# YukeWang96/GNNAdvisor_OSDI21

Hardware: AMD Instinct MI355X
Metric: aggregated edges/sec, GCN sum-aggregation SpMM (SAG) hidden=64 (higher is better)
Workload: dtype f32; 1 GPU; reddit-like power-law graph, random node order; num_nodes=232965, nnz=114623790, dim=64, partSize=128, num_parts=1008217, parallelism=single GPU, call=GNNA.SAG (pybind module, reference signature, fresh output), decider=auto/mi355x, column_phases=16, build_id=0.6.1+df1c895dd0a4406b

## Files before the change

### gnnadvisor_osdi21_amd/_lib.py

```python
from __future__ import annotations

import ctypes
import math
import os

import torch

_HERE = os.path.dirname(os.path.abspath(__file__))
LIB_PATH = os.environ.get("GNNA_LIB") or os.path.join(_HERE, "csrc", "libgnna.so")

GNNA_OK = 0


class GnnaError(RuntimeError):
    pass


class Tuning(ctypes.Structure):
    _fields_ = [("struct_size", ctypes.c_int), ("groups_per_chunk", ctypes.c_int), ("loads_in_flight", ctypes.c_int),
                ("blocks_per_cu", ctypes.c_int), ("xcd_remap", ctypes.c_int),
                ("trust_canonical", ctypes.c_int), ("column_phases", ctypes.c_int),
                ("avg_degree", ctypes.c_int), ("nonlocal_ids", ctypes.c_int), ("gcn_prescale", ctypes.c_int),
                ("pad_rows", ctypes.c_int), ("zero_fill", ctypes.c_int),
                ("sweep", ctypes.c_int), ("sweep_slack", ctypes.c_int), ("deterministic", ctypes.c_int),
# ... 47 lines not shown
    "gnna_release_graph": (i, [p]), "gnna_forget_graph": (i, [p]), "gnna_forget_plans": (i, [p]),
    "gnna_runtime_counters": (None, [pi64]),
    "gnna_runtime_counters_ex": (i, [pi64, i]),
    "gnna_debug_untrusted_copies": (i, [p]),
    "gnna_profile_begin": (i, [i]),
    "gnna_profile_end": (i, [pd, pd, pi]),
    "gnna_agg_edge_ld_f32": (i, [p, i64, i64, p, p, p, p, p] + _SIZES),
    "gnna_edge_softmax_f32": (i, [p, p, i64, i64, i, p, p]),
    "gnna_edge_softmax_backward_f32": (i, [p, p, p, i64, i64, i, p, p]),
    "gnna_reverse_edges_i32": (i, [p, p, i64, p]),
    "gnna_agg_reduce_ld_f32": (i, [i, p, i64, i64, p, p, p, p, i64, p] + _SIZES),
    "gnna_scatter_arg_ld_f32": (i, [p, i64, p, i64, p, i64, p, i64, i64, i, u, p]),
    "gnna_gat_forward_f32": (i, _GAT_FWD + [i64, i, i, i64, i, u, p]),
    "gnna_gat_forward_rect_f32": (i, _GAT_FWD + [i64, i64, i, i, i64, i, u, p]),
    "gnna_gat_backward_f32": (i, _GAT_BWD + [p, p, p, p, f, p, i64, p, p, i64, i, i, i64, i, u, p]),
    "gnna_gat_backward_dir_f32": (i, _GAT_BWD + _GAT_BOTH + [i64, i, i, i, u, p]),
    "gnna_gat_backward_rect_f32": (i, _GAT_BWD + _GAT_BOTH + [i64, i64, i, i, i, u, p]),
    "gnna_transpose_csr_i32": (i, [p, p, i64, i64, p, p, p, p]),
    "gnna_count_parts_device_i32": (i64, [i, p, i64, p]),
    "gnna_build_part_device_i32": (i, [i, p, i64, p, p, i64, p]),
    "gnna_sample_neighbors_i32": (i, [p, p, i64, p, i64, i, u64, i, p, p, p, p, p, p, i64, i64, pi64, p]),
    "gnna_agg_typed_expand_ld_f32": (i, _TYPED),
    "gnna_agg_typed_contract_ld_f32": (i, _TYPED),
    "gnna_typed_coef_grad_ld_f32": (i, [p, i64, i64, p, i64, i64, p, p, p, p, p, p, i, i, i, i64, i, u, p]),
}
EXT_SIGNATURES = {
    "gnna_gat_forward_drop_f32": (i, _GAT_FWD[:9] + [f, u64] + _GAT_FWD[9:] + [i64, i64, i, i, i64, i, u, p]),
    "gnna_gat_backward_drop_f32": (i, _GAT_BWD + _GAT_BOTH[:11] + [f, u64] + _GAT_BOTH[11:] + [i64, i64, i, i, i, u, p]),
}
_GRAPH_T = ([p] * 4 + [i64]) * 2
GATV2_SIGNATURES = {
    "gnna_gatv2_forward_f32": (i, [p, i64, p, i64, p] + [p] * 4 + [f, f, u64, p, i64, p, i64, i64, i, i, i64, i, u, p]),
    "gnna_gatv2_backward_f32": (i, [p, i64, p, i64, p, p, p, i64, p, i64] + _GRAPH_T + [f, f, u64, p, i64, p, i64, p,
                                                                                       i64, i64, i, i, i, u, p]),
}
DOTATTN_SIGNATURES = {
    "gnna_dot_attn_forward_f32": (i, [p, i64] * 3 + [p] * 4 + [f, f, u64, p, i64, p, i64, i64, i, i, i64, i, u, p]),
    "gnna_dot_attn_backward_f32": (i, [p, i64] * 3 + [p, p, i64, p, i64] + _GRAPH_T + [f, f, u64] + [p, i64] * 3 +
                                   [i64, i64, i, i, i, u, p]),
}
GATEDGE_SIGNATURES = {
    "gnna_gat_edge_forward_f32": (i, _GAT_FWD[:4] + [p] + _GAT_FWD[4:9] + [f, u64] + _GAT_FWD[9:] + [i64, i64, i64, i, i, i64, i, u, p]),
    "gnna_gat_edge_backward_f32": (i, _GAT_BWD[:4] + [p] + _GAT_BWD[4:] + _GAT_BOTH[:10] + [p, f, f, u64] + _GAT_BOTH[11:] +
                                   [p, i64, i64, i64, i, i, i, u, p]),
    "gnna_gat_alpha_f32": (i, [p] * 6 + [f, p, i64, i64, i64, i, p]),
}
STATS_SIGNATURES = {
    "gnna_agg_stats_ld_f32": (i, [p, i64, i64, p, p, p] + [p, i64] * 6 + [i64, i, i64, i, u, p]),
}
SOFTAGG_SIGNATURES = {
    "gnna_agg_softmax_ld_f32": (i, [p, i64, i64, p, i, p, p] + [p, i64] * 3 + [i64, i, u, p]),
    "gnna_agg_softmax_backward_ld_f32": (i, [p, i64, i64, p, i] + [p, i64] * 3 + [p, p, p, i64, i64, i, u, p]),
}
del p, i, i64, u, u64, f, s, pd, pi, pi64
EXPORTS = tuple(SIGNATURES)
EXT_EXPORTS = tuple(EXT_SIGNATURES)
GATV2_EXPORTS = tuple(GATV2_SIGNATURES)
DOTATTN_EXPORTS = tuple(DOTATTN_SIGNATURES)
SIGNATURE_TABLES = (SIGNATURES, EXT_SIGNATURES, GATV2_SIGNATURES, DOTATTN_SIGNATURES)
GATEDGE_EXPORTS = tuple(GATEDGE_SIGNATURES)
STATS_EXPORTS = tuple(STATS_SIGNATURES)
LATER_SIGNATURE_TABLES = (GATEDGE_SIGNATURES, STATS_SIGNATURES)
SOFTAGG_EXPORTS = tuple(SOFTAGG_SIGNATURES)
NEWER_SIGNATURE_TABLES = (SOFTAGG_SIGNATURES,)


def load() -> ctypes.CDLL:
    global _lib
    if _lib is not None:
        return _lib
    if not os.path.exists(LIB_PATH):
        raise ImportError(
            f"{LIB_PATH} is missing: the HIP extension has not been built "
            "(run `python -m gnnadvisor_osdi21_amd.build`). There is no CPU fallback.")
    L = ctypes.CDLL(LIB_PATH)
    for table in SIGNATURE_TABLES + LATER_SIGNATURE_TABLES + NEWER_SIGNATURE_TABLES:
        for name, (restype, argtypes) in table.items():
            fn = getattr(L, name)
            fn.restype = restype
            if argtypes is not None:
                fn.argtypes = argtypes
    _lib = L
    return L


def _check(rc: int) -> None:
    if rc != GNNA_OK:
        raise GnnaError(f"libgnna error {rc}: {load().gnna_last_error().decode()}")


def _ptr(t: torch.Tensor | None) -> int | None:
    return None if t is None else t.data_ptr()


def _stream(device: torch.device) -> int:
    return torch.cuda.current_stream(device).cuda_stream


def _call(device, fn_name: str, *args) -> None:
    with torch.cuda.device(device):
        _check(getattr(load(), fn_name)(*args, _stream(device)))


def _need_device(t: torch.Tensor, what: str) -> None:
    if not t.is_cuda:
        raise GnnaError(f"{what} needs device tensors: there is no CPU path in libgnna")


def set_tuning(groups_per_chunk=-1, loads_in_flight=-1, blocks_per_cu=-1, xcd_remap=-1,
               trust_canonical=-1, column_phases=-1, avg_degree=-1, nonlocal_ids=-1, gcn_prescale=-1,
               pad_rows=-1, zero_fill=-1, sweep=-1, sweep_slack=-1, deterministic=-1, pack_ids=-1,
               wide_blocks=-1, ids_check_every=-1) -> None:
    t = Tuning(ctypes.sizeof(Tuning), groups_per_chunk, loads_in_flight, blocks_per_cu, xcd_remap, trust_canonical, column_phases,
               avg_degree, nonlocal_ids, gcn_prescale, pad_rows, zero_fill, sweep, sweep_slack, deterministic,
               pack_ids, ids_check_every, wide_blocks)
    _check(load().gnna_set_tuning(ctypes.byref(t)))


def reset_tuning() -> None:
    _check(load().gnna_set_tuning(None))


def device_cus() -> int:
    return int(load().gnna_device_cus())


def host_threads() -> int:
    return int(load().gnna_host_threads())

# ... 88 lines not shown


def degrees(row_pointers: torch.Tensor) -> torch.Tensor:
    rp = _host_i32(row_pointers)
    out = torch.empty(rp.numel() - 1, dtype=torch.float32)
    _check(load().gnna_degrees_f32(rp.data_ptr(), rp.numel() - 1, out.data_ptr()))
    return out


def edge_span(src, dst) -> float:
    s, d = _host_i32(src), _host_i32(dst)
    v = ctypes.c_double()
    _check(load().gnna_edge_span(s.data_ptr(), d.data_ptr(), s.numel(), ctypes.byref(v)))
    return v.value


def _reorder(entry: str, src, dst, num_nodes: int) -> torch.Tensor:
    s, d = _host_i32(src), _host_i32(dst)
    out = torch.empty(int(num_nodes), dtype=torch.int32)
    _check(getattr(load(), entry)(s.data_ptr(), d.data_ptr(), s.numel(), int(num_nodes), out.data_ptr()))
    return out


def reorder_rcm(src, dst, num_nodes: int) -> torch.Tensor:
    return _reorder("gnna_reorder_rcm_i32", src, dst, num_nodes)


def reorder_community(src, dst, num_nodes: int) -> torch.Tensor:
    return _reorder("gnna_reorder_community_i32", src, dst, num_nodes)


def reorder_community_csr(row_pointers, column_index, num_nodes: int) -> torch.Tensor:
    rp, ci = _host_i32(row_pointers), _host_i32(column_index)
    assert rp.numel() == int(num_nodes) + 1
    out = torch.empty(int(num_nodes), dtype=torch.int32)
    _check(load().gnna_reorder_community_csr_i32(rp.data_ptr(), ci.data_ptr(), int(num_nodes), out.data_ptr()))
    return out


def relabel_edges_(src: torch.Tensor, dst: torch.Tensor, new_id: torch.Tensor, num_nodes: int) -> float:
    for t in (src, dst, new_id):
        assert t.dtype == torch.int32 and t.is_contiguous() and not t.is_cuda
    v = ctypes.c_double()
    _check(load().gnna_relabel_edges_i32(src.data_ptr(), dst.data_ptr(), src.numel(), new_id.data_ptr(), int(num_nodes), ctypes.byref(v)))
    return v.value


def relabel_csr(row_pointers, column_index, new_id, num_nodes: int):
    rp, ci, nid = _host_i32(row_pointers), _host_i32(column_index), _host_i32(new_id)
    out_rp = torch.empty(int(num_nodes) + 1, dtype=torch.int32)
    out_ci = torch.empty(max(1, ci.numel()), dtype=torch.int32)
    _check(load().gnna_relabel_csr_i32(rp.data_ptr(), ci.data_ptr(), int(num_nodes), nid.data_ptr(), out_rp.data_ptr(), out_ci.data_ptr()))
    return out_rp, out_ci[:ci.numel()]


def last_num_phases() -> int:
    return int(load().gnna_last_num_phases())


def last_num_launches() -> int:
    return int(load().gnna_last_num_launches())


def profile_begin(max_calls: int) -> None:
    _check(load().gnna_profile_begin(int(max_calls)))


def profile_end() -> dict:
    a, b, n = ctypes.c_double(), ctypes.c_double(), ctypes.c_int()
    _check(load().gnna_profile_end(ctypes.byref(a), ctypes.byref(b), ctypes.byref(n)))
    return dict(main_ms=a.value, prologue_ms=b.value, calls=n.value)


def count_parts(partSize: int, indptr: torch.Tensor) -> int:
    assert indptr.dtype == torch.int32 and not indptr.is_cuda and indptr.is_contiguous()
    n = load().gnna_count_parts(int(partSize), indptr.data_ptr(), indptr.numel() - 1)
    if n < 0:
        _check(int(n))
    return int(n)


def build_part(partSize: int, indptr: torch.Tensor):
    indptr = indptr.contiguous()
    P = count_parts(partSize, indptr)
    pp = torch.empty(P + 1, dtype=torch.int32)
    p2n = torch.empty(P, dtype=torch.int32)
    _check(load().gnna_build_part_i32(int(partSize), indptr.data_ptr(), indptr.numel() - 1,
                                      pp.data_ptr(), p2n.data_ptr(), P))
    return pp, p2n


def _fresh_output(shape, device, dtype=torch.float32) -> torch.Tensor:
    if os.environ.get("GNNA_DEBUG_POISON", "0") not in ("", "0"):
        return torch.full(tuple(shape), float("nan") if dtype.is_floating_point else -(2 ** 31), dtype=dtype, device=device)
    return torch.empty(tuple(shape), dtype=dtype, device=device)


def _agg(fn_name, X, row_pointers, column_index, extra, part_pointers, part2Node, partSize, dimWorker,
         warpPerBlock, out):
    _need_device(X, "aggregation")
    assert X.dtype == torch.float32 and X.is_contiguous() and X.dim() == 2
    for t in (column_index, part_pointers, part2Node):
        assert t.dtype == torch.int32 and t.is_contiguous() and t.device == X.device
    if out is None:
        out = _fresh_output(X.shape, X.device)
    _call(X.device, fn_name, X.data_ptr(), _ptr(row_pointers), column_index.data_ptr(), extra,
# ... 821 lines not shown
```

### gnnadvisor_osdi21_amd/build.py

```python
from __future__ import annotations

import os
import subprocess
import sys
import sysconfig

PKG = os.path.dirname(os.path.abspath(__file__))
ROOT = os.path.dirname(PKG)
CSRC = os.path.join(PKG, "csrc")
INCLUDE = os.path.join(ROOT, "include")
LIB = os.path.join(CSRC, "libgnna.so")
EXT = os.path.join(PKG, "GNNAdvisor.so")
ARCH = "gfx950"
HIPCC = os.environ.get("HIPCC", "/opt/rocm/bin/hipcc")

LIB_SOURCES = [os.path.join(CSRC, f) for f in ("gnna_agg.hip", "gnna_stream.hip", "gnna_sweep.hip", "gnna_x16.hip", "gnna_reduce.hip", "gnna_stats.hip", "gnna_softagg.hip", "gnna_sddmm.hip", "gnna_edge.hip", "gnna_gat.hip", "gnna_gatv2.hip", "gnna_dotattn.hip", "gnna_typed.hip", "gnna_transpose.hip", "gnna_sample.hip",
                                                "gnna_gemm.hip", "gnna_runtime.hip", "gnna_host.cpp", "gnna_reorder.cpp")]
LIB_DEPS = LIB_SOURCES + [os.path.join(CSRC, "gnna_internal.h"), os.path.join(CSRC, "gnna_device.h"), os.path.join(CSRC, "gnna_launch.h"),
                           os.path.join(CSRC, "gnna_gat_common.h"), os.path.join(CSRC, "gnna_keys.h"), os.path.join(INCLUDE, "gnna.h"), os.path.join(INCLUDE, "gnna_ext.h"),
                           os.path.join(INCLUDE, "gnna_gatv2.h"), os.path.join(INCLUDE, "gnna_dotattn.h"),
                           os.path.join(INCLUDE, "gnna_gat_edge.h"), os.path.join(INCLUDE, "gnna_stats.h"),
                           os.path.join(INCLUDE, "gnna_softagg.h")]
EXT_SOURCES = [os.path.join(CSRC, "gnna_torch.cpp")]
EXT_DEPS = EXT_SOURCES + [os.path.join(INCLUDE, "gnna.h"), os.path.join(INCLUDE, "gnna_ext.h"), os.path.join(INCLUDE, "gnna_gatv2.h"),
                          os.path.join(INCLUDE, "gnna_dotattn.h"), os.path.join(INCLUDE, "gnna_gat_edge.h"),
                          os.path.join(INCLUDE, "gnna_stats.h"), os.path.join(INCLUDE, "gnna_softagg.h")]


def source_hash() -> str:
    import hashlib
    h = hashlib.sha256()
    for path in sorted(set(LIB_DEPS + EXT_DEPS)):
        h.update(os.path.relpath(path, ROOT).encode() + b"\0")
        with open(path, "rb") as f:
            h.update(f.read())
        h.update(b"\0")
    return h.hexdigest()[:16]


def _stale(target: str, deps: list[str]) -> bool:
    if not os.path.exists(target):
        return True
    t = os.path.getmtime(target)
    return any(os.path.getmtime(d) > t for d in deps)


def build_lib(force: bool = False, verbose: bool = False) -> str:
    from concurrent.futures import ThreadPoolExecutor
    objdir = os.path.join(CSRC, "build")
    os.makedirs(objdir, exist_ok=True)
    headers = [d for d in LIB_DEPS if d not in LIB_SOURCES]
    flags = [f"--offload-arch={ARCH}", "-O3", "-std=c++17", "-fPIC", "-munsafe-fp-atomics", "-ffp-contract=off",
             "-fvisibility=hidden", "-I" + INCLUDE, "-I" + CSRC]
    jobs, objs = [], []
    digest = source_hash()
    stamp = os.path.join(objdir, "source_hash.txt")
    stamped = open(stamp).read().strip() if os.path.exists(stamp) else ""
    if not force and stamped == digest and os.path.exists(LIB) and not _stale(LIB, LIB_DEPS):
        return LIB
    for src in LIB_SOURCES:
        obj = os.path.join(objdir, os.path.basename(src) + ".o")
        objs.append(obj)
        carries_id = os.path.basename(src) == "gnna_host.cpp"
        if force or _stale(obj, [src] + headers) or (carries_id and stamped != digest):
            jobs.append([HIPCC, *flags, *([f'-DGNNA_SOURCE_HASH="{digest}"'] if carries_id else []), "-c", src, "-o", obj])

    def run(cmd):
        if verbose:
            print(" ".join(cmd), flush=True)
        subprocess.check_call(cmd)
    if jobs:
        with ThreadPoolExecutor(max_workers=min(len(jobs), os.cpu_count() or 4)) as pool:
            list(pool.map(run, jobs))
    if jobs or force or _stale(LIB, objs):
        run([HIPCC, f"--offload-arch={ARCH}", "-shared", "-fPIC", "-fvisibility=hidden", *objs, "-o", LIB])
# ... 45 lines not shown
```

### gnnadvisor_osdi21_amd/csrc/gnna_agg.hip

```cpp
#include <hip/hip_runtime.h>

#include <algorithm>
#include <cmath>
#include <cstdint>
#include <cstdio>

#include "gnna.h"
#include "gnna_device.h"
#include "gnna_internal.h"

namespace gnna {
namespace {


__global__ void __launch_bounds__(kBlock)
prologue_kernel(float *__restrict__ Y, size_t n_floats, int D, int ldy, const int32_t *__restrict__ p2n,
                const int32_t *__restrict__ pp, int64_t P, int32_t *flag, int32_t seq, int validate, int zero_fill,
                const int32_t *__restrict__ chk_ids, int64_t chk_n, const unsigned long long *__restrict__ chk_sum,
                int32_t *stale_flag, uint32_t *__restrict__ clear_words, int n_clear)
{
    if (blockIdx.x == 0 && (int)threadIdx.x < n_clear) clear_words[threadIdx.x] = 0u;
    const unsigned fill_blocks = chk_ids ? gridDim.x - 1 : gridDim.x;
    if (blockIdx.x >= fill_blocks) {
        if (threadIdx.x < kWave) {
// ... 560 lines not shown
                                              "stream capture: run the sequence once before capturing it");
        if (plan.stats.unsorted > 0)
            return fail(GNNA_ERR_UNSUPPORTED, "windowed aggregation: the column ids of %.0f neighbor-groups are not in increasing "
                                              "order (sort the ids of every row, as the loader's CSR has them)", plan.stats.unsorted);
        cnt = plan.cnt; S = plan.S; B = 1;
        win_lo = win_begin; win_hi = win_end == num_windows ? S : win_end;
    } else {
        if (tune.column_phases >= 2 && num_in_rows >= kMaxSlices) {
            B = std::min(tune.column_phases, kMaxSlices);
            rc = get_slice_plan(ds, stream, column_index, part_pointers, part2Node, num_parts, num_in_rows, false, false, &plan);
            if (rc != GNNA_OK) return rc;
        } else if (tune.column_phases == 0 && can_slice && foot_bytes >= ((size_t)6 << 20)) {
            rc = get_slice_plan(ds, stream, column_index, part_pointers, part2Node, num_parts, num_in_rows, true, false, &plan);
            if (rc != GNNA_OK) return rc;
            if (plan.cnt && plan.stats.valid)
                B = choose_slices(plan.stats, foot_bytes, plan.S, plan.slice_rows, num_nodes, num_in_rows == num_nodes,
                                  tune.nonlocal_ids == 1);
        }
        cnt = plan.cnt;
        if (cnt) S = plan.S;
        if (!cnt || B < 2) { B = 1; cnt = nullptr; }
    }

    const int auto_Bs = (cnt && !windowed && plan.stats.valid)
                            ? sweep_auto_phases(tune, mode, dim, foot_bytes, num_nodes, num_in_rows, plan.stats, B, ds->num_cus,
                                                tune.deterministic == 1, partSize) : 0;
    if (mode != MODE_EDGE && cnt && !windowed && dim >= 4 && (tune.sweep == 1 || auto_Bs > 0) && tune.deterministic != 1 &&
        sweep_supports(mode, dim, x_bytes)) {
        int Bs = B;
        if (auto_Bs > 0) {
            Bs = std::min(auto_Bs, S);
        } else if (tune.column_phases < 2) {
            Bs = std::max(2, std::min(std::min(std::min(16, 2 * B), std::max(2, partSize / 4)), S));
        }
        const int32_t *sw_ids = nullptr; const uint32_t *sw_off = nullptr;
        if (plan.handle && (tune.pack_ids == 1 || (tune.pack_ids == 0 && plan.pinned)) && tune.xcd_remap != 0) {
            rc = get_packed_ids(ds, stream, plan.handle, Bs, kWave, true, false, &sw_ids, &sw_off, &chk_sum, &chk_n, stale_flag, seq,
                                tune.ids_check_every);
            if (rc != GNNA_OK) return rc;
            if (sw_ids) count_event(CTR_PACKED_LAUNCHES);
        }
        uint32_t *sync = ds->sweep_sync + (size_t)call_block_of(ds, stream, seq) * kSweepSlotWords;
        static_assert(kXcds * 16 + 2 <= kBlock, "the prologue clears the sweep counters with one block");
        rc = run_prologue(0, sync, kXcds * 16 + 2);
        if (rc != GNNA_OK) return rc;
        SweepLaunch w;
        w.mode = mode; w.X = X; w.col = column_index; w.pp = part_pointers; w.p2n = part2Node; w.Y = out;
        w.cnt = cnt; w.row_scale = row_scale; w.flag = flag; w.seq = seq; w.trust = tune.trust_canonical ? 1 : 0; w.sync = sync;
        w.P = num_parts; w.D = dim; w.ldx = ldx; w.ldy = ldy; w.S = S; w.B = Bs;
        w.relu = relu; w.num_out_rows = num_nodes;
        w.U = std::max(tune.loads_in_flight, 8);
        w.rows_with_edges = plan.stats.valid ? (int64_t)std::min((double)num_nodes, plan.stats.groups) : num_nodes;
        if (tune.groups_per_chunk > 64) w.rounds = tune.groups_per_chunk / 64;
        w.slack = tune.sweep_slack; w.wgs_per_cu = tune.blocks_per_cu;
        w.dynamic = tune.xcd_remap != 0;
        w.plain_ok = !accumulate_into_out; w.eps = eps;
        w.ids_packed = sw_ids; w.item_off = sw_off; w.packed_stale = stale_flag;
        t_last_phases = Bs;
        t_last_launches = 1;
        rc = launch_sweep(ds, w, stream);
        if (rc != GNNA_OK) return rc;
        profile_record(prof_call, 2, stream);
        return GNNA_OK;
    }

    int G = std::min(64, tune.groups_per_chunk * B);
    if (mode == MODE_EDGE && cnt && !windowed && plan.handle && plan.pinned && (plan.stats.valid || tune.sweep == 1) &&
        tune.xcd_remap != 0) {
        const int Bs = sweep_phases_of_width(tune, dim, foot_bytes, x_bytes, num_nodes, num_in_rows, plan.stats, B, ds->num_cus,
                                             partSize, S);
        if (Bs >= 2) { B = Bs; G = kWave; }
    }
    t_last_phases = B;
    StreamLaunch a;
    a.mode = mode; a.X = X; a.col = column_index; a.pp = part_pointers; a.p2n = part2Node; a.Y = out;
    a.cnt = cnt; a.row_scale = row_scale; a.flag = flag; a.seq = seq;
    if (mode == MODE_EDGE) { a.deg_row = nullptr; a.deg_col = nullptr; a.edge_w = degrees_in; }
    else { a.deg_row = degrees; a.deg_col = degrees_in; }
    a.trust = tune.trust_canonical ? 1 : 0; a.P = num_parts;
    a.D = dim; a.ldx = ldx; a.ldy = ldy; a.G = G; a.U = tune.loads_in_flight; a.S = S; a.B = B;
    a.win_lo = win_lo; a.win_hi = win_hi; a.relu = relu; a.num_out_rows = num_nodes;
    t_last_launches = 1;
    a.wide = wide; a.plain_ok = (B == 1 && !accumulate_into_out && !windowed); a.xcd_remap = tune.xcd_remap != 0;
    a.eps = eps;
    if (tune.deterministic == 1 && !windowed) {
        const int G_eff = std::max(1, std::min(a.G, kWave));
        const size_t chunks = (size_t)((num_parts + G_eff - 1) / G_eff);
        const size_t part_bytes = ((chunks * 2 * (size_t)dim * sizeof(float)) + 255) & ~(size_t)255;
        const size_t stamp_bytes = chunks * 2 * sizeof(int32_t);
        void *ws = nullptr;
        rc = get_workspace(ds, stream, 2, part_bytes + stamp_bytes, &ws);
        if (rc != GNNA_OK) return rc;
        a.det = true;
        a.det_part = static_cast<float *>(ws);
        a.det_stamp = reinterpret_cast<int32_t *>(static_cast<char *>(ws) + part_bytes);
        hipError_t em = hipMemsetAsync(a.det_stamp, 0, stamp_bytes, stream);
        if (em != hipSuccess) return fail(GNNA_ERR_HIP, "deterministic schedule scratch: %s", hipGetErrorString(em));
        t_last_launches = B;
    }
    if (cnt && !windowed && plan.handle && (tune.pack_ids == 1 || (tune.pack_ids == 0 && plan.pinned))) {
        rc = get_packed_ids(ds, stream, plan.handle, B, std::max(1, std::min(a.G, kWave)), true, false, &a.ids_packed, &a.item_off,
                            &chk_sum, &chk_n, stale_flag, seq, tune.ids_check_every);
        a.packed_stale = stale_flag;
        if (rc != GNNA_OK) return rc;
        if (a.ids_packed) count_event(CTR_PACKED_LAUNCHES);
    }
    const bool sparse = !a.det && a.plain_ok && tune.zero_fill != 2 &&
// ... 292 lines not shown
```

### gnnadvisor_osdi21_amd/csrc/gnna_internal.h

```cpp
#ifndef GNNA_INTERNAL_H_
#define GNNA_INTERNAL_H_

#include <hip/hip_runtime.h>

#include <atomic>
#include <cstddef>
#include <cstdint>
#include <map>
#include <utility>
#include <vector>

#include "gnna.h"
#include "gnna_launch.h"

namespace gnna {

int fail(int code, const char *fmt, ...) __attribute__((format(printf, 2, 3)));

int host_thread_budget(int cap);

void apply_graph_hints(const void *column_index, int dim, gnna_tuning *tune);

int launch_ok(const char *prefix_fmt, ...) __attribute__((format(printf, 1, 2)));
inline int xcd_remap_on()
// ... 98 lines not shown
       CTR_COUNT = 10 };
void count_event(int which);

struct StreamLaunch {
    int mode;
    const float *X; const int32_t *col; const int32_t *pp; const int32_t *p2n; float *Y;
    const uint8_t *cnt;
    const float *row_scale;
    const float *deg_row; const float *deg_col;
    const float *A = nullptr;
    const float *edge_w = nullptr;
    const int32_t *flag; int32_t seq; int32_t trust;
    int64_t P;
    int D, ldx, G, U, S, B;
    int lda = 0;
    int ldy = 0;
    int win_lo = 0, win_hi = 0;
    bool relu = false;
    int64_t num_out_rows = 0;
    bool wide, plain_ok, xcd_remap;
    float eps;
    bool det = false;
    float *det_part = nullptr; int32_t *det_stamp = nullptr;
    const int32_t *ids_packed = nullptr; const uint32_t *item_off = nullptr;
    const int32_t *packed_stale = nullptr;
};
int launch_stream(const StreamLaunch &a, hipStream_t stream);
int launch_stream_epilogue_only(const StreamLaunch &a, hipStream_t stream);

struct SweepLaunch {
    int mode;
    const float *X; const int32_t *col; const int32_t *pp; const int32_t *p2n; float *Y;
    const uint8_t *cnt;
    const float *row_scale;
    const int32_t *flag; int32_t seq; int32_t trust;
    uint32_t *sync;
    int64_t P;
    int D, ldx, U, S, B;
    int ldy = 0;
    bool relu = false;
    int64_t num_out_rows = 0;
    int rounds = 0;
    int64_t rows_with_edges = 0;
    int slack = 0;
    int wgs_per_cu = 0;
    bool dynamic = true;
    bool plain_ok;
    float eps;
    const int32_t *ids_packed = nullptr; const uint32_t *item_off = nullptr;
    const int32_t *packed_stale = nullptr;
};
bool sweep_supports(int mode, int dim, size_t x_bytes);
int sweep_acc_rows(int dim, int wgs_per_cu);
int launch_sweep(DeviceState *ds, const SweepLaunch &a, hipStream_t stream);
int sweep_auto_phases(const gnna_tuning &t, int mode, int dim, size_t x_bytes, int64_t num_out_rows, int64_t num_in_rows,
                      const SlicePlanStats &st, int B, int num_cus, bool deterministic, int part_size);
constexpr int kSweepListCap = 1023;
constexpr int kSweepSlotWords = 8 * 16 + 2 + 2 * kSweepListCap;

struct X16Launch {
    int mode;
    int in_type, out_type;
    const void *input; int64_t ld_in, num_in_rows;
    const int32_t *column_index; const float *degrees_out; const float *degrees_in; float epsilon;
    const int32_t *part_pointers; const int32_t *part2Node;
    void *out; int64_t ld_out, num_out_rows;
    int dim; int64_t num_parts; int partSize;
    bool accumulate, relu, xcd_remap;
    int prof_call = -1;
};
int launch_x16(DeviceState *ds, hipStream_t stream, const X16Launch &c);
int reserve_x16(DeviceState *ds, hipStream_t stream, int64_t num_in_rows, int64_t num_out_rows, int dim);
int launch_zero_fill(DeviceState *ds, hipStream_t stream, float *out, int64_t rows, int dim, int64_t ld);
void launch_relu_rows(DeviceState *ds, hipStream_t stream, float *out, int64_t rows, int dim, int64_t ld);

int64_t scan_tiles(int64_t n);
int launch_exclusive_scan(hipStream_t stream, int32_t *data, int64_t n, int32_t *partial);
int refuse_capture(const char *what, hipStream_t stream);

int profile_acquire_call(bool has_work);
void profile_record(int call, int which, hipStream_t stream);

}

#endif
```

### gnnadvisor_osdi21_amd/csrc/gnna_sweep.hip

```cpp
#include <hip/hip_runtime.h>

#include <algorithm>
#include <cmath>
#include <cstdint>

#include "gnna.h"
#include "gnna_device.h"
#include "gnna_internal.h"

namespace gnna {
namespace {

constexpr int kSweepIdSlots = 512;
constexpr int kSweepBlock = 1024;
constexpr int kSweepWaves = kSweepBlock / kWave;
constexpr int kSweepLockWords = 128;

template <int LPR, int WGS> constexpr int acc_floats()
{
    return WGS == 1 ? (LPR >= 16 ? 32768 : 28672) : (LPR >= 16 ? 15360 : 11264);
}

__device__ __forceinline__ void lds_add(float *p, float v)
{
    typedef __attribute__((address_space(3))) float lds_float;
    (void)__hip_atomic_fetch_add((lds_float *)p, v, __ATOMIC_RELAXED, __HIP_MEMORY_SCOPE_WORKGROUP);
}

struct SweepParams {
    const float *X;
    const int32_t *col;
    const int32_t *pp;
    const int32_t *p2n;
    float *Y;
    const uint8_t *cnt;
    const float *row_scale;
    const int32_t *flag;
    uint32_t *sync;
    int64_t P;
    int32_t seq;
    int32_t trust;
    int32_t D;
    int32_t ldx;
    int32_t ldy;
    int32_t relu;
    int32_t S;
    int32_t B;
    int32_t rounds;
    int32_t plain_ok;
    int32_t dynamic;
    int32_t slack;
    float eps;
    const int32_t *ids_packed;
    const uint32_t *item_off;
    const int32_t *packed_stale;
    int64_t num_chunks;
};

__device__ __forceinline__ int64_t lower_bound64(const int32_t *__restrict__ pp, int64_t P, int64_t target, int lane)
{
    int64_t lo = 0, hi = P;
    while (hi > lo) {
        const int64_t span = hi - lo;
        const int64_t idx = lo + (span * lane) / kWave;
        const bool below = (int64_t)pp[idx] < target;
        const int c = __popcll(__ballot(below));
        if (c == 0) { hi = lo; break; }
        const int64_t new_lo = lo + (span * (c - 1)) / kWave + 1;
        const int64_t new_hi = c < kWave ? lo + (span * c) / kWave : hi;
        lo = new_lo;
        hi = new_hi > new_lo ? new_hi : new_lo;
    }
    return lo;
}

__device__ __forceinline__ int64_t sweep_set_start(int64_t i, int64_t num_sets, int64_t nnz, const int32_t *__restrict__ pp,
                                                   int64_t P, bool canonical, bool align64, int lane)
{
    const int64_t target = i >= num_sets ? nnz : (nnz * i) / num_sets;
    int64_t g = i <= 0 ? 0 : (i >= num_sets ? P : (canonical ? lower_bound64(pp, P, target, lane) : (P * i) / num_sets));
    if (align64 && g < P) g &= ~(int64_t)(kWave - 1);
    return g;
}

__global__ void __launch_bounds__(kBlock)
sweep_relu_fixup_kernel(float *__restrict__ Y, int64_t N, int D, int ldy, const uint32_t *__restrict__ list,
                        const int32_t *flag, int32_t seq, int32_t trust, int whole)
{
    const int lane = threadIdx.x & (kWave - 1);
    const int64_t wave = ((int64_t)blockIdx.x * blockDim.x + threadIdx.x) >> 6;
    const int64_t nwaves = ((int64_t)gridDim.x * blockDim.x) >> 6;
    const bool canonical = trust || (*flag != seq);
    auto clamp_row = [&](int64_t r) {
        float *row = Y + (size_t)r * (size_t)ldy;
        for (int i = lane; i < D; i += kWave) row[i] = fmaxf(row[i], 0.f);
    };
    if (whole || !canonical || list[1] != 0u) {
        for (int64_t r = wave; r < N; r += nwaves) clamp_row(r);
        return;
    }
    const uint32_t n = list[0] < (uint32_t)kSweepListCap ? list[0] : (uint32_t)kSweepListCap;
    for (int64_t i = wave; i < (int64_t)n; i += nwaves) {
        const int64_t first = (int64_t)list[2 + 2 * i], cnt = (int64_t)list[3 + 2 * i];
        for (int64_t r = first; r < first + cnt && r < N; r++) clamp_row(r);
    }
}

template <int LPR, int MODE, int U, int WGS>
__global__ void __launch_bounds__(kSweepBlock) __attribute__((amdgpu_waves_per_eu(4 * WGS, 4 * WGS)))
sweep_kernel(const SweepParams p)
{
    typedef typename VecOf<4>::T VT;
    typedef typename VecOf<4>::M MT;
    constexpr int RPI = kWave / LPR;
    constexpr int RL = (kSweepIdSlots / RPI < kWave) ? kSweepIdSlots / RPI : kWave;
    static_assert(RL % U == 0, "a round is a whole number of batches");
    constexpr int ACC = acc_floats<LPR, WGS>();
    __shared__ float s_acc[ACC];
    __shared__ uint32_t s_off[kSweepWaves][RL * RPI];
    __shared__ int64_t s_g[2];
    __shared__ int s_ctl[8];
    __shared__ unsigned s_lock[kSweepLockWords];

    const int lane = threadIdx.x & (kWave - 1);
    const int wib = __builtin_amdgcn_readfirstlane((int)threadIdx.x >> 6);
    const int lslot = lane / LPR;
    const int c = lane % LPR;
    const int D = p.D;
    const bool canonical = p.trust || (*p.flag != p.seq);
    const bool stale_ids = p.ids_packed != nullptr && *p.packed_stale == p.seq;
    const char *xbase = reinterpret_cast<const char *>(p.X);
    const uint32_t row_bytes32 = (uint32_t)p.ldx * 4u;
    uint32_t *offs = s_off[wib];
    const int CAP = ACC / D;
    const unsigned long long upto = (2ull << lane) - 1ull;
    const unsigned long long above = ~upto;

    const int piece = c * 4;
    const bool cvalid = piece < D;
    int dcol = piece, shift = 0;
    if (piece + 4 > D && cvalid) { dcol = D - 4; shift = piece - dcol; }
    const uint32_t col_off = (uint32_t)(cvalid ? dcol : 0) * 4u;
    const int comp = lane >> 4;
    const bool add_lane = LPR <= 16 ? ((lane & 15) < LPR && cvalid && comp >= shift) : (lslot == 0 && cvalid);

    const int xcd = (int)(blockIdx.x & (kXcds - 1));
    const int nbx = (int)(gridDim.x >> 3);
    const int bx = (int)(blockIdx.x >> 3);
    uint32_t *ctr = p.sync + xcd * 16;
    const bool syncing = p.slack < 1000 && nbx > 1;
    const int B = p.B, R = p.rounds;
    const int64_t nnz = (int64_t)p.pp[p.P];
    const int64_t num_sets = (int64_t)gridDim.x * R;

    if (threadIdx.x == 0) { s_ctl[2] = 0; s_ctl[3] = 0; }

    for (int r = 0; r < R; r++) {
        const int64_t set = ((int64_t)xcd * nbx + bx) * R + r;
        if (wib < 2) {
            const int64_t g = sweep_set_start(set + wib, num_sets, nnz, p.pp, p.P, canonical, p.ids_packed != nullptr, lane);
            if (lane == 0) s_g[wib] = g;
        }
        if (threadIdx.x == 0) { s_ctl[0] = 0; s_ctl[1] = 0; }
        __syncthreads();
        const int64_t g_lo = s_g[0], g_hi = s_g[1];
        int row_first = 0, row_last = -1, set_prev_row = -1, set_next_row = -1;
        if (g_hi > g_lo) {
            row_first = p.p2n[g_lo];
            row_last = p.p2n[g_hi - 1];
            if (g_lo > 0) set_prev_row = p.p2n[g_lo - 1];
            if (g_hi < p.P) set_next_row = p.p2n[g_hi];
        }
        int nrows = 0;
        if (canonical && row_last >= row_first) nrows = row_last - row_first + 1 < CAP ? row_last - row_first + 1 : CAP;
        if (p.relu && canonical && threadIdx.x == 0 && g_hi > g_lo) {
            uint32_t *list = p.sync + kXcds * 16;
            auto push = [&](int first, int cnt) {
                const uint32_t idx = atomicAdd(&list[0], 1u);
                if (idx < (uint32_t)kSweepListCap) { list[2 + 2 * idx] = (uint32_t)first; list[3 + 2 * idx] = (uint32_t)cnt; }
                else list[1] = 1u;
            };
            if (set_prev_row == row_first) push(row_first, 1);
            const int over_rows = row_last - row_first + 1 - CAP;
            if (over_rows > 2048) list[1] = 1u;
            else
                for (int r0 = 0; r0 < over_rows; r0 += 16) push(row_first + CAP + r0, over_rows - r0 < 16 ? over_rows - r0 : 16);
        }
        for (int i = threadIdx.x; i < nrows * D; i += kSweepBlock) s_acc[i] = 0.f;
        __syncthreads();
// ... 36 lines not shown
                            if (lane == 0) __hip_atomic_store(&s_ctl[2], (int)now, __ATOMIC_RELAXED, __HIP_MEMORY_SCOPE_WORKGROUP);
                            break;
                        }
                        if (wall_clock64() - t0 > 20000ull) {
                            if (lane == 0) __hip_atomic_store(&s_ctl[3], 1, __ATOMIC_RELAXED, __HIP_MEMORY_SCOPE_WORKGROUP);
                            break;
                        }
                        __builtin_amdgcn_s_sleep(4);
                    }
                }
            }
            last_T = T;
            int wave_prev_row = -1, wave_next_row = -1;
            if (ng > 0) {
                const int64_t lo = dyn ? g0 : gw_lo, hi = dyn ? g0 + ng : gw_hi;
                if (lo > g_lo) wave_prev_row = p.p2n[lo - 1];
                if (hi < g_hi) wave_next_row = p.p2n[hi];
            }
            if (dyn && lane == 0) {
                const unsigned bit = 1u << (chunk & 31);
                while (__hip_atomic_fetch_or(&s_lock[chunk >> 5], bit, __ATOMIC_ACQUIRE, __HIP_MEMORY_SCOPE_WORKGROUP) & bit)
                    __builtin_amdgcn_s_sleep(2);
            }

            if (ng > 0)
            {
                const int f_lo = t * p.S / B, f_hi = (t + 1) * p.S / B;

                const bool gl = lane < ng;
                const int my_row = gl ? p.p2n[g0 + lane] : -1;
                const int pa = gl ? p.pp[g0 + lane] : 0;
                const int pb = gl ? p.pp[g0 + lane + 1] : 0;
                int cum_lo = 0, cum_hi = 0x7fffffff;
                if (gl) {
                    if (f_lo > 0) cum_lo = p.cnt[(size_t)(f_lo - 1) * (size_t)p.P + (size_t)(g0 + lane)];
                    if (f_hi < p.S) cum_hi = p.cnt[(size_t)(f_hi - 1) * (size_t)p.P + (size_t)(g0 + lane)];
                }
                const bool packed = dyn && p.ids_packed != nullptr && !stale_ids;
                const uint32_t item_base = packed ? p.item_off[(size_t)t * (size_t)p.num_chunks + (size_t)(g0 >> 6)] : 0u;
                const int32_t *__restrict__ ids = packed ? p.ids_packed : p.col;
                const int len = pb > pa ? pb - pa : 0;
                const int beg = cum_lo < len ? cum_lo : len;
                int end = cum_hi < len ? cum_hi : len;
                end = end > beg ? end : beg;
                const int n_own = gl ? end - beg : 0;
                if (__ballot(n_own > 0) != 0) {
                    const int up_row = __shfl_up(my_row, 1);
                    const bool seg_start = gl && (lane == 0 || my_row != up_row || !canonical);
                    const unsigned long long SS = __ballot(seg_start);
                    const int up_end = __shfl_up(pa + end, 1), up_n = __shfl_up(n_own, 1);
                    const bool cont = n_own > 0 && !seg_start && up_n > 0 && (packed || up_end == pa + beg);
                    const unsigned long long NE = __ballot(n_own > 0 && !cont);
                    const int n_cum = wave_inclusive_scan(n_own);
                    const unsigned long long heads_above = NE & above;
                    const int next_head = heads_above ? __builtin_ctzll(heads_above) : 64;
                    const int chain_cum = __shfl(n_cum, next_head - 1);
                    const int n = (n_own > 0 && !cont) ? chain_cum - n_cum + n_own : 0;
                    const unsigned long long between = SS & above & (next_head < 63 ? ((2ull << next_head) - 1ull) : ~0ull);
                    const bool last_in_seg = n > 0 && (next_head == 64 || between != 0);
                    const int aslot = my_row - row_first;
                    const int over = (aslot < 0 || aslot >= nrows) ? 1 : 0;
                    const int edge = (my_row == wave_prev_row || my_row == wave_next_row) ? 4 : 0;

                    const int rank = __popcll(NE & (upto >> 1));
                    const int Rn = __popcll(NE);
                    const int dstl = (n > 0 ? rank : 63) << 2;
                    const int c_pbeg = __builtin_amdgcn_ds_permute(dstl, packed ? (int)item_base + (n_cum - n_own) : pa + beg);
                    const int t_n = __builtin_amdgcn_ds_permute(dstl, n);
                    const int c_n = lane < Rn ? t_n : 0;
                    const int c_meta = __builtin_amdgcn_ds_permute(dstl, ((over ? my_row : aslot) << 3) | edge | (last_in_seg ? 2 : 0) | over);
                    const int c_nl = (c_n + RPI - 1) / RPI;
                    const int c_offI = wave_inclusive_scan(c_nl);
                    const int c_offX = c_offI - c_nl;
                    const int L = __builtin_amdgcn_readlane(c_offI, kWave - 1);

                    VT acc = vzero<4>();
                    struct Round {
                        uint32_t o[RPI];
                        int v_j, k_meta;
                        unsigned long long FL, TM;
                        int nr;
                    };
                    auto describe = [&](int r0) -> Round {
                        Round rd;
                        const unsigned long long below = __ballot(lane < Rn && c_offI <= r0);
                        unsigned long long inwin = __ballot(lane < Rn && c_offI > r0 && c_offI <= r0 + RL - 1);
                        unsigned long long E = 0;
                        while (inwin) {
                            const int kk = __builtin_ctzll(inwin);
                            inwin &= inwin - 1;
                            E |= 1ull << (__builtin_amdgcn_readlane(c_offI, kk) - r0);
                        }
                        const int kp = __popcll(below) + __popcll(E & upto);
                        const int k_offX = __shfl(c_offX, kp), k_pbeg = __shfl(c_pbeg, kp), k_n = __shfl(c_n, kp);
                        rd.k_meta = __shfl(c_meta, kp);
                        const int J = r0 + lane;
                        const bool active = J < L && lane < RL;
                        const int i = J - k_offX;
                        const int e_j = k_pbeg + i * RPI;
                        int v_j = active ? k_n - i * RPI : 0;
                        const bool fl_j = active && (rd.k_meta & 2) && v_j <= RPI;
                        v_j = v_j > RPI ? RPI : v_j;
                        rd.v_j = v_j;
                        rd.FL = __ballot(fl_j);
                        rd.TM = __ballot(active && v_j < RPI);
                        rd.nr = (L - r0) < RL ? (L - r0) : RL;
#pragma unroll
                        for (int q = 0; q < RPI; q++) rd.o[q] = 0u;
                        if (lane < RL) {
                            if (v_j == RPI) {
                                if constexpr (RPI >= 4) {
                                    typedef int i32x4 __attribute__((ext_vector_type(4)));
                                    typedef i32x4 i32x4u __attribute__((aligned(4)));
#pragma unroll
                                    for (int s4 = 0; s4 < RPI; s4 += 4) {
                                        const i32x4 tt = *reinterpret_cast<const i32x4u *>(ids + e_j + s4);
                                        rd.o[s4] = (uint32_t)tt[0]; rd.o[s4 + 1] = (uint32_t)tt[1]; rd.o[s4 + 2] = (uint32_t)tt[2]; rd.o[s4 + 3] = (uint32_t)tt[3];
                                    }
                                } else {
#pragma unroll
                                    for (int q = 0; q < RPI; q++) rd.o[q] = (uint32_t)ids[e_j + q];
                                }
                            } else {
                                const uint32_t first = v_j > 0 ? (uint32_t)ids[e_j] : 0u;
#pragma unroll
                                for (int q = 0; q < RPI; q++) {
                                    rd.o[q] = first;
                                    if (q > 0 && q < v_j) rd.o[q] = (uint32_t)ids[e_j + q];
                                }
                            }
                        }
                        return rd;
                    };
                    Round cur = describe(0);
                    for (int r0 = 0; r0 < L; r0 += RL) {
                        if (lane < RL) {
#pragma unroll
                            for (int q = 0; q < RPI; q++) offs[lane * RPI + q] = cur.o[q] * row_bytes32;
                        }
                        const bool more = r0 + RL < L;
                        Round nxt = cur;
                        if (more) nxt = describe(r0 + RL);
                        const int v_j = cur.v_j, k_meta = cur.k_meta, nr = cur.nr;
                        const unsigned long long FL = cur.FL, TM = cur.TM;

                        auto row_ptr = [&](uint32_t o) -> const MT * {
// ... 67 lines not shown
                                consume(u, b * U + u);
                                v[u] = *row_ptr(nn[u]);
                            }
                        }
#pragma unroll
                        for (int u = 0; u < U; u++) {
                            const int j = (nb - 1) * U + u;
                            if (j < nr) consume(u, j);
                        }
                        cur = nxt;
                    }
                }
            }
            if (dyn && lane == 0)
                (void)__hip_atomic_fetch_and(&s_lock[chunk >> 5], ~(1u << (chunk & 31)), __ATOMIC_RELEASE, __HIP_MEMORY_SCOPE_WORKGROUP);
            if (syncing && lane == 0 && (dyn || chunk == per_step - 1)) {
                const int done = __hip_atomic_fetch_add(&s_ctl[1], 1, __ATOMIC_RELAXED, __HIP_MEMORY_SCOPE_WORKGROUP) + 1;
                if (done % (dyn ? nchunks : kSweepWaves) == 0)
                    (void)__hip_atomic_fetch_add(ctr, 1u, __ATOMIC_RELAXED, __HIP_MEMORY_SCOPE_AGENT);
            }
        }
        if (dyn && nchunks == 0 && syncing && threadIdx.x == 0)
            (void)__hip_atomic_fetch_add(ctr, (uint32_t)B, __ATOMIC_RELAXED, __HIP_MEMORY_SCOPE_AGENT);
        __syncthreads();

        for (int q = wib; q < nrows; q += kSweepWaves) {
            const int row = row_first + q;
            const bool shared = row == set_prev_row || row == set_next_row;
            const bool use_atomic = shared || !p.plain_ok;
            float scale = 1.f;
            if constexpr (MODE == MODE_GIN) {
                scale = p.eps;
                if (p.row_scale) scale *= p.row_scale[row];
            }
            float *dst = p.Y + (size_t)row * (size_t)p.ldy;
            const float *src = s_acc + q * D;
            for (int i = lane; i < D; i += kWave) {
                const float val = src[i] * scale;
                if (!use_atomic) __builtin_nontemporal_store(p.relu ? fmaxf(val, 0.f) : val, dst + i);
                else unsafeAtomicAdd(dst + i, val);
            }
        }
        __syncthreads();
    }
}

typedef void (*SweepKernel)(const SweepParams);

template <int LPR, int MODE, int WGS>
SweepKernel pick_sweep_u(int u)
{
    constexpr int RPI = kWave / LPR;
    constexpr int RL = (kSweepIdSlots / RPI < kWave) ? kSweepIdSlots / RPI : kWave;
    if constexpr (RL % 16 == 0 && WGS == 1) {
        if (u >= 16) return sweep_kernel<LPR, MODE, 16, WGS>;
    }
    if constexpr (RL % 8 == 0 && WGS == 1) {
        if (u >= 8) return sweep_kernel<LPR, MODE, 8, WGS>;
    }
    return sweep_kernel<LPR, MODE, 4, WGS>;
}

template <int MODE, int WGS>
SweepKernel pick_sweep(int lpr, int u)
{
    switch (lpr) {
    case 4: return pick_sweep_u<4, MODE, WGS>(u);
    case 8: return pick_sweep_u<8, MODE, WGS>(u);
    case 16: return pick_sweep_u<16, MODE, WGS>(u);
    default: return pick_sweep_u<32, MODE, WGS>(u);
    }
}

}

int sweep_acc_rows(int dim, int wgs)
{
    const int pieces = (dim + 3) / 4;
    const int acc = wgs == 1 ? (pieces <= 8 ? acc_floats<8, 1>() : acc_floats<16, 1>())
                             : (pieces <= 8 ? acc_floats<8, 2>() : acc_floats<16, 2>());
    return std::max(1, acc / std::max(1, dim));
}

bool sweep_supports(int mode, int dim, size_t x_bytes)
{
    return (mode == MODE_SAG || mode == MODE_GIN) && dim >= 4 && dim <= 128 && x_bytes <= 0xffffffffull;
}

int launch_sweep(DeviceState *ds, const SweepLaunch &a, hipStream_t stream)
{
    SweepParams p;
    p.X = a.X; p.col = a.col; p.pp = a.pp; p.p2n = a.p2n; p.Y = a.Y; p.cnt = a.cnt; p.row_scale = a.row_scale;
    p.flag = a.flag; p.seq = a.seq; p.trust = a.trust; p.sync = a.sync;
    p.P = a.P; p.D = a.D; p.ldx = a.ldx; p.S = a.S; p.B = a.B; p.plain_ok = a.plain_ok ? 1 : 0; p.eps = a.eps;
    p.ldy = a.ldy > 0 ? a.ldy : a.D;
    p.relu = (a.relu && a.plain_ok) ? 1 : 0;
    p.slack = a.slack > 0 ? a.slack : 2;
    p.ids_packed = a.packed_stale ? a.ids_packed : nullptr; p.item_off = a.item_off; p.packed_stale = a.packed_stale;
    p.num_chunks = (a.P + kWave - 1) / kWave;
    p.dynamic = a.dynamic ? 1 : 0;
    int lpr = 4;
    const int pieces = (a.D + 3) / 4;
    while (lpr < 32 && lpr < pieces) lpr <<= 1;
    const int wgs = a.wgs_per_cu == 2 ? 2 : 1;
    SweepKernel k = wgs == 1 ? (a.mode == MODE_GIN ? pick_sweep<MODE_GIN, 1>(lpr, a.U) : pick_sweep<MODE_SAG, 1>(lpr, a.U))
                             : (a.mode == MODE_GIN ? pick_sweep<MODE_GIN, 2>(lpr, a.U) : pick_sweep<MODE_SAG, 2>(lpr, a.U));
    const int cus_per_xcd = std::max(1, ds->num_cus / kXcds);
    const unsigned grid = (unsigned)(cus_per_xcd * kXcds * wgs);
    const int cap = sweep_acc_rows(a.D, wgs);
    int R = a.rounds;
    if (R <= 0) {
        const double rows = (double)std::max<int64_t>(1, a.rows_with_edges);
        R = (int)std::max(1.0, std::ceil(rows / ((double)grid * 0.9 * (double)cap)));
    }
    p.rounds = std::min(R, 4096);
    hipLaunchKernelGGL(k, dim3(grid), dim3(kSweepBlock), 0, stream, p);
    hipError_t e = hipGetLastError();
    if (e != hipSuccess) return fail(GNNA_ERR_HIP, "sweep launch: %s", hipGetErrorString(e));
    count_event(CTR_SWEEP_LAUNCHES);
    if (a.relu) {
        const bool whole = !a.plain_ok;
        const int64_t blocks = std::max<int64_t>(1, std::min<int64_t>((a.num_out_rows + kWavesPerBlock - 1) / kWavesPerBlock, 256 * 8));
        hipLaunchKernelGGL(sweep_relu_fixup_kernel, dim3((unsigned)blocks), dim3(kBlock), 0, stream, a.Y, a.num_out_rows, a.D, p.ldy,
                           a.sync + kXcds * 16, a.flag, a.seq, a.trust, whole ? 1 : 0);
        e = hipGetLastError();
        if (e != hipSuccess) return fail(GNNA_ERR_HIP, "epilogue launch: %s", hipGetErrorString(e));
    }
    return GNNA_OK;
}

}
```

Baseline: 82.99 billion edges/s.

## Resize sweep kernel for two workgroups per CU and expose LDS sizing queries

Makes the sweep kernel's block size depend on workgroups per CU: 16 waves with one workgroup, 12 waves with two. The LDS accumulator size is now derived from the LDS budget minus the per-wave id slots, so two workgroups can fill the CU. The U=16 unroll variant is removed, a U=2 variant is added for the two-workgroup case, and the lane-mask arithmetic is rewritten with mbcnt. It also adds C/Python queries for accumulator rows and LDS bytes. With the default single workgroup per CU the main effects are losing U=16 and the cheaper mask code, so the default path may slow down if it relied on U=16.

Measured after the change: 82.85 billion edges/s, median of 2. About the same (-0.2%).

```diff
diff --git a/gnnadvisor_osdi21_amd/_lib.py b/gnnadvisor_osdi21_amd/_lib.py
--- a/gnnadvisor_osdi21_amd/_lib.py
+++ b/gnnadvisor_osdi21_amd/_lib.py
@@ -123,6 +123,10 @@
     "gnna_agg_softmax_ld_f32": (i, [p, i64, i64, p, i, p, p] + [p, i64] * 3 + [i64, i, u, p]),
     "gnna_agg_softmax_backward_ld_f32": (i, [p, i64, i64, p, i] + [p, i64] * 3 + [p, p, p, i64, i64, i, u, p]),
 }
+SWEEP_SIGNATURES = {
+    "gnna_sweep_acc_rows": (i, [i, i]),
+    "gnna_sweep_lds_bytes": (i, [i, i]),
+}
 del p, i, i64, u, u64, f, s, pd, pi, pi64
 EXPORTS = tuple(SIGNATURES)
 EXT_EXPORTS = tuple(EXT_SIGNATURES)
@@ -134,6 +138,7 @@
 LATER_SIGNATURE_TABLES = (GATEDGE_SIGNATURES, STATS_SIGNATURES)
 SOFTAGG_EXPORTS = tuple(SOFTAGG_SIGNATURES)
 NEWER_SIGNATURE_TABLES = (SOFTAGG_SIGNATURES,)
+SWEEP_EXPORTS = tuple(SWEEP_SIGNATURES)
 
 
 def load() -> ctypes.CDLL:
@@ -145,7 +150,7 @@
             f"{LIB_PATH} is missing: the HIP extension has not been built "
             "(run `python -m gnnadvisor_osdi21_amd.build`). There is no CPU fallback.")
     L = ctypes.CDLL(LIB_PATH)
-    for table in SIGNATURE_TABLES + LATER_SIGNATURE_TABLES + NEWER_SIGNATURE_TABLES:
+    for table in SIGNATURE_TABLES + LATER_SIGNATURE_TABLES + NEWER_SIGNATURE_TABLES + (SWEEP_SIGNATURES,):
         for name, (restype, argtypes) in table.items():
             fn = getattr(L, name)
             fn.restype = restype
@@ -340,6 +345,18 @@
     out_ci = torch.empty(max(1, ci.numel()), dtype=torch.int32)
     _check(load().gnna_relabel_csr_i32(rp.data_ptr(), ci.data_ptr(), int(num_nodes), nid.data_ptr(), out_rp.data_ptr(), out_ci.data_ptr()))
     return out_rp, out_ci[:ci.numel()]
+
+
+def sweep_acc_rows(dim: int, workgroups_per_cu: int = 1) -> int:
+    rows = int(load().gnna_sweep_acc_rows(dim, workgroups_per_cu))
+    _check(min(rows, 0))
+    return rows
+
+
+def sweep_lds_bytes(dim: int, workgroups_per_cu: int = 1) -> int:
+    n = int(load().gnna_sweep_lds_bytes(dim, workgroups_per_cu))
+    _check(min(n, 0))
+    return n
 
 
 def last_num_phases() -> int:
diff --git a/gnnadvisor_osdi21_amd/build.py b/gnnadvisor_osdi21_amd/build.py
--- a/gnnadvisor_osdi21_amd/build.py
+++ b/gnnadvisor_osdi21_amd/build.py
@@ -20,7 +20,7 @@
                            os.path.join(CSRC, "gnna_gat_common.h"), os.path.join(CSRC, "gnna_keys.h"), os.path.join(INCLUDE, "gnna.h"), os.path.join(INCLUDE, "gnna_ext.h"),
                            os.path.join(INCLUDE, "gnna_gatv2.h"), os.path.join(INCLUDE, "gnna_dotattn.h"),
                            os.path.join(INCLUDE, "gnna_gat_edge.h"), os.path.join(INCLUDE, "gnna_stats.h"),
-                           os.path.join(INCLUDE, "gnna_softagg.h")]
+                           os.path.join(INCLUDE, "gnna_softagg.h"), os.path.join(INCLUDE, "gnna_sweep.h")]
 EXT_SOURCES = [os.path.join(CSRC, "gnna_torch.cpp")]
 EXT_DEPS = EXT_SOURCES + [os.path.join(INCLUDE, "gnna.h"), os.path.join(INCLUDE, "gnna_ext.h"), os.path.join(INCLUDE, "gnna_gatv2.h"),
                           os.path.join(INCLUDE, "gnna_dotattn.h"), os.path.join(INCLUDE, "gnna_gat_edge.h"),
diff --git a/gnnadvisor_osdi21_amd/csrc/gnna_agg.hip b/gnnadvisor_osdi21_amd/csrc/gnna_agg.hip
--- a/gnnadvisor_osdi21_amd/csrc/gnna_agg.hip
+++ b/gnnadvisor_osdi21_amd/csrc/gnna_agg.hip
@@ -636,7 +636,7 @@
         w.U = std::max(tune.loads_in_flight, 8);
         w.rows_with_edges = plan.stats.valid ? (int64_t)std::min((double)num_nodes, plan.stats.groups) : num_nodes;
         if (tune.groups_per_chunk > 64) w.rounds = tune.groups_per_chunk / 64;
-        w.slack = tune.sweep_slack; w.wgs_per_cu = tune.blocks_per_cu;
+        w.slack = tune.sweep_slack; w.wgs_per_cu = tune.blocks_per_cu == 2 ? 2 : 1;
         w.dynamic = tune.xcd_remap != 0;
         w.plain_ok = !accumulate_into_out; w.eps = eps;
         w.ids_packed = sw_ids; w.item_off = sw_off; w.packed_stale = stale_flag;
diff --git a/gnnadvisor_osdi21_amd/csrc/gnna_internal.h b/gnnadvisor_osdi21_amd/csrc/gnna_internal.h
--- a/gnnadvisor_osdi21_amd/csrc/gnna_internal.h
+++ b/gnnadvisor_osdi21_amd/csrc/gnna_internal.h
@@ -174,6 +174,7 @@
 };
 bool sweep_supports(int mode, int dim, size_t x_bytes);
 int sweep_acc_rows(int dim, int wgs_per_cu);
+int sweep_lds_bytes(int dim, int wgs_per_cu);
 int launch_sweep(DeviceState *ds, const SweepLaunch &a, hipStream_t stream);
 int sweep_auto_phases(const gnna_tuning &t, int mode, int dim, size_t x_bytes, int64_t num_out_rows, int64_t num_in_rows,
                       const SlicePlanStats &st, int B, int num_cus, bool deterministic, int part_size);
diff --git a/gnnadvisor_osdi21_amd/csrc/gnna_sweep.hip b/gnnadvisor_osdi21_amd/csrc/gnna_sweep.hip
--- a/gnnadvisor_osdi21_amd/csrc/gnna_sweep.hip
+++ b/gnnadvisor_osdi21_amd/csrc/gnna_sweep.hip
@@ -5,6 +5,7 @@
 #include <cstdint>
 
 #include "gnna.h"
+#include "gnna_sweep.h"
 #include "gnna_device.h"
 #include "gnna_internal.h"
 
@@ -12,14 +13,29 @@
 namespace {
 
 constexpr int kSweepIdSlots = 512;
-constexpr int kSweepBlock = 1024;
-constexpr int kSweepWaves = kSweepBlock / kWave;
 constexpr int kSweepLockWords = 128;
 
+constexpr int sweep_waves(int wgs) { return wgs == 1 ? 16 : 12; }
+constexpr int sweep_waves_per_simd(int wgs) { return wgs * sweep_waves(wgs) / 4; }
+
+constexpr int sweep_slot_bytes(int lpr)
+{
+    const int rpi = kWave / lpr;
+    const int rl = (kSweepIdSlots / rpi < kWave) ? kSweepIdSlots / rpi : kWave;
+    return rl * rpi * 4;
+}
+
 template <int LPR, int WGS> constexpr int acc_floats()
 {
-    return WGS == 1 ? (LPR >= 16 ? 32768 : 28672) : (LPR >= 16 ? 15360 : 11264);
-}
+    constexpr int slots = sweep_waves(WGS) * sweep_slot_bytes(LPR >= 16 ? 16 : 8);
+    return ((WGS == 1 ? 144 : 77) * 1024 - slots) / 4;
+}
+static_assert(acc_floats<16, 1>() == 32768 && acc_floats<8, 1>() == 28672, "the one-workgroup form is unchanged");
+static_assert(acc_floats<16, 2>() == 16640 && acc_floats<8, 2>() == 13568, "two workgroups fill the CU");
+constexpr int kSweepCtlBytes = 16 + 32 + kSweepLockWords * 4;
+static_assert(2 * (acc_floats<16, 2>() * 4 + sweep_waves(2) * sweep_slot_bytes(16) + kSweepCtlBytes) <= 160 * 1024 &&
+              2 * (acc_floats<8, 2>() * 4 + sweep_waves(2) * sweep_slot_bytes(8) + kSweepCtlBytes) <= 160 * 1024,
+              "two workgroups' LDS fits the CU");
 
 __device__ __forceinline__ void lds_add(float *p, float v)
 {
@@ -107,9 +123,12 @@
 }
 
 template <int LPR, int MODE, int U, int WGS>
-__global__ void __launch_bounds__(kSweepBlock) __attribute__((amdgpu_waves_per_eu(4 * WGS, 4 * WGS)))
+__global__ void __launch_bounds__(sweep_waves(WGS) * kWave)
+__attribute__((amdgpu_waves_per_eu(sweep_waves_per_simd(WGS), sweep_waves_per_simd(WGS))))
 sweep_kernel(const SweepParams p)
 {
+    constexpr int kSweepWaves = sweep_waves(WGS);
+    constexpr int kSweepBlock = kSweepWaves * kWave;
     typedef typename VecOf<4>::T VT;
     typedef typename VecOf<4>::M MT;
     constexpr int RPI = kWave / LPR;
@@ -133,8 +152,10 @@
     const uint32_t row_bytes32 = (uint32_t)p.ldx * 4u;
     uint32_t *offs = s_off[wib];
     const int CAP = ACC / D;
-    const unsigned long long upto = (2ull << lane) - 1ull;
-    const unsigned long long above = ~upto;
+    auto count_below = [](unsigned long long m) -> int {
+        return (int)__builtin_amdgcn_mbcnt_hi((unsigned)(m >> 32), __builtin_amdgcn_mbcnt_lo((unsigned)m, 0u));
+    };
+    auto bits_above = [&](unsigned long long m) -> unsigned long long { return (m >> lane) >> 1; };
 
     const int piece = c * 4;
     const bool cvalid = piece < D;
@@ -277,17 +298,17 @@
                     const bool cont = n_own > 0 && !seg_start && up_n > 0 && (packed || up_end == pa + beg);
                     const unsigned long long NE = __ballot(n_own > 0 && !cont);
                     const int n_cum = wave_inclusive_scan(n_own);
-                    const unsigned long long heads_above = NE & above;
-                    const int next_head = heads_above ? __builtin_ctzll(heads_above) : 64;
+                    const unsigned long long heads_above = bits_above(NE);
+                    const int next_head = heads_above ? lane + 1 + __builtin_ctzll(heads_above) : 64;
                     const int chain_cum = __shfl(n_cum, next_head - 1);
                     const int n = (n_own > 0 && !cont) ? chain_cum - n_cum + n_own : 0;
-                    const unsigned long long between = SS & above & (next_head < 63 ? ((2ull << next_head) - 1ull) : ~0ull);
+                    const unsigned long long between = next_head < 64 ? bits_above(SS) << (63 - (next_head - lane - 1)) : 0ull;
                     const bool last_in_seg = n > 0 && (next_head == 64 || between != 0);
                     const int aslot = my_row - row_first;
                     const int over = (aslot < 0 || aslot >= nrows) ? 1 : 0;
                     const int edge = (my_row == wave_prev_row || my_row == wave_next_row) ? 4 : 0;
 
-                    const int rank = __popcll(NE & (upto >> 1));
+                    const int rank = count_below(NE);
                     const int Rn = __popcll(NE);
                     const int dstl = (n > 0 ? rank : 63) << 2;
                     const int c_pbeg = __builtin_amdgcn_ds_permute(dstl, packed ? (int)item_base + (n_cum - n_own) : pa + beg);
@@ -316,7 +337,7 @@
                             inwin &= inwin - 1;
                             E |= 1ull << (__builtin_amdgcn_readlane(c_offI, kk) - r0);
                         }
-                        const int kp = __popcll(below) + __popcll(E & upto);
+                        const int kp = __popcll(below) + count_below(E) + (int)((E >> lane) & 1ull);
                         const int k_offX = __shfl(c_offX, kp), k_pbeg = __shfl(c_pbeg, kp), k_n = __shfl(c_n, kp);
                         rd.k_meta = __shfl(c_meta, kp);
                         const int J = r0 + lane;
@@ -490,13 +511,11 @@
 {
     constexpr int RPI = kWave / LPR;
     constexpr int RL = (kSweepIdSlots / RPI < kWave) ? kSweepIdSlots / RPI : kWave;
-    if constexpr (RL % 16 == 0 && WGS == 1) {
-        if (u >= 16) return sweep_kernel<LPR, MODE, 16, WGS>;
-    }
     if constexpr (RL % 8 == 0 && WGS == 1) {
         if (u >= 8) return sweep_kernel<LPR, MODE, 8, WGS>;
     }
-    return sweep_kernel<LPR, MODE, 4, WGS>;
+    if constexpr (WGS == 2 && LPR <= 8) return sweep_kernel<LPR, MODE, 2, WGS>;
+    else return sweep_kernel<LPR, MODE, 4, WGS>;
 }
 
 template <int MODE, int WGS>
@@ -518,6 +537,16 @@
     const int acc = wgs == 1 ? (pieces <= 8 ? acc_floats<8, 1>() : acc_floats<16, 1>())
                              : (pieces <= 8 ? acc_floats<8, 2>() : acc_floats<16, 2>());
     return std::max(1, acc / std::max(1, dim));
+}
+
+int sweep_lds_bytes(int dim, int wgs)
+{
+    const int pieces = (dim + 3) / 4;
+    int lpr = 4;
+    while (lpr < 32 && lpr < pieces) lpr <<= 1;
+    const int acc = wgs == 1 ? (lpr <= 8 ? acc_floats<8, 1>() : acc_floats<16, 1>())
+                             : (lpr <= 8 ? acc_floats<8, 2>() : acc_floats<16, 2>());
+    return acc * 4 + sweep_waves(wgs == 1 ? 1 : 2) * sweep_slot_bytes(lpr) + kSweepCtlBytes;
 }
 
 bool sweep_supports(int mode, int dim, size_t x_bytes)
@@ -552,7 +581,7 @@
         R = (int)std::max(1.0, std::ceil(rows / ((double)grid * 0.9 * (double)cap)));
     }
     p.rounds = std::min(R, 4096);
-    hipLaunchKernelGGL(k, dim3(grid), dim3(kSweepBlock), 0, stream, p);
+    hipLaunchKernelGGL(k, dim3(grid), dim3(sweep_waves(wgs) * kWave), 0, stream, p);
     hipError_t e = hipGetLastError();
     if (e != hipSuccess) return fail(GNNA_ERR_HIP, "sweep launch: %s", hipGetErrorString(e));
     count_event(CTR_SWEEP_LAUNCHES);
@@ -568,3 +597,20 @@
 }
 
 }
+
+extern "C" {
+#pragma GCC visibility push(default)
+int gnna_sweep_acc_rows(int dim, int workgroups_per_cu)
+{
+    if (dim < 1 || workgroups_per_cu < 1 || workgroups_per_cu > 2)
+        return gnna::fail(GNNA_ERR_INVALID_ARGUMENT, "gnna_sweep_acc_rows: dim >= 1 and 1 or 2 workgroups per CU");
+    return gnna::sweep_acc_rows(dim, workgroups_per_cu);
+}
+int gnna_sweep_lds_bytes(int dim, int workgroups_per_cu)
+{
+    if (dim < 1 || workgroups_per_cu < 1 || workgroups_per_cu > 2)
+        return gnna::fail(GNNA_ERR_INVALID_ARGUMENT, "gnna_sweep_lds_bytes: dim >= 1 and 1 or 2 workgroups per CU");
+    return gnna::sweep_lds_bytes(dim, workgroups_per_cu);
+}
+#pragma GCC visibility pop
+}
diff --git a/include/gnna_sweep.h b/include/gnna_sweep.h
--- /dev/null
+++ b/include/gnna_sweep.h
@@ -0,0 +1,17 @@
+#ifndef GNNA_SWEEP_H_
+#define GNNA_SWEEP_H_
+
+#include "gnna.h"
+
+#ifdef __cplusplus
+extern "C" {
+#endif
+
+GNNA_API int gnna_sweep_acc_rows(int dim, int workgroups_per_cu);
+GNNA_API int gnna_sweep_lds_bytes(int dim, int workgroups_per_cu);
+
+#ifdef __cplusplus
+}
+#endif
+
+#endif
```
